# feifeibear/long-context-attention

Hardware: AMD Instinct MI355X
Metric: attention TFLOP/s (algorithmic, causal fwd+bwd) + iter ms of LongContextAttention at seqlen 64K, ulysses x ring (higher is better)
Workload: dtype bf16

## Files before the change

long-context-attention_amd/csrc/usp_flash_bwd_dq64.hip:

```cpp
#include <stdlib.h>

#include <type_traits>

#include "usp_bwd_params.hpp"
#include "usp_common.hpp"
#include "usp_hip.h"
#include "usp_mfma64.hpp"

namespace usp {

#ifndef USP_Q64_PF
#define USP_Q64_PF 3
#endif
constexpr int kQ64_PF = USP_Q64_PF;
#ifndef USP_Q64_Y1
#define USP_Q64_Y1 24
#endif
constexpr int kQ64_Y1 = USP_Q64_Y1;

#ifdef USP_Q64_TIMING
#define USP_TM(...) __VA_ARGS__
#else
#define USP_TM(...)
#endif

template <int DT, bool CAUSAL>
__global__ __launch_bounds__(256, 1) void flash_bwd_dq64_kernel(const BwdParams ) {
  using E = Elem<DT>;
  using M = M64<DT>;
  constexpr int D = 128, kBM = 256;
  constexpr int ROWB = D * 2;
  constexpr int TILEB = kTile * ROWB;
  constexpr int VOFF = 2 * TILEB;
  constexpr int NKT = D / 16, NDJ = D / 32;
  constexpr int PF = kQ64_PF;

  extern __shared__ __attribute__((aligned(16))) char smem_raw[];
  if ((uint32_t)(uintptr_t)(USP_LDS char*)smem_raw != 0u) __builtin_trap();
  USP_LDS char* smem = (USP_LDS char*)(uintptr_t)0;

  const int tid = threadIdx.x;
  const int lane = tid & 63;
  const int wave = __builtin_amdgcn_readfirstlane(tid >> 6);
  const int l31 = lane & 31;
  const int hi = lane >> 5;
  typedef const __attribute__((address_space(4))) BwdParams* KArgs;
  KArgs p = (KArgs)__builtin_amdgcn_kernarg_segment_ptr();
  asm volatile("" : "+s"(p));

  const int dma_row = lane >> 4;
  const int dma_c8 = ((lane & 15) ^ ((lane >> 4) << 2)) * 16;
  const int k_voff = dma_row * (int)p->k_ss * 2 + dma_c8, v_voff = dma_row * (int)p->v_ss * 2 + dma_c8;
  const int rd_base = l31 * ROWB + ((hi ^ tile_swz<D>(l31)) * 16);
  int tr_addr[NDJ][2];
  {
    const int i = lane & 15, grp = (lane >> 4) & 1;
#pragma unroll
    for (int dj = 0; dj < NDJ; ++dj)
#pragma unroll
      for (int e = 0; e < 2; ++e) {
        const int rr = 8 * e + 4 * hi + (i >> 2);
        const int slot = 4 * dj + 2 * grp + ((i & 3) >> 1);
        tr_addr[dj][e] = rr * ROWB + ((slot ^ tile_swz<D>(rr)) * 16) + (i & 1) * 8;
      }
  }
  const float c = p->scale_log2;

  const ItemWalk walk(p->n_items);
  for (int pass = 0;; ++pass) {
  int w = walk.at(pass);
  if (w < 0) break;
  asm volatile("" : "+s"(p));
  USP_TM(const uint64_t tm_item = __builtin_amdgcn_s_memtime();)
  w = walk.dealt(w, p->nblk);
  if (p->ksplit <= 1) w = walk.grouped(w, p->nblk, p->walk_g);
  const int qt_r = w % p->nblk;
  int rest = w / p->nblk;
  const int qt = CAUSAL ? (p->nblk - 1 - qt_r) : qt_r;
  int cut = 0;
  if (p->ksplit > 1) { cut = rest % p->ksplit; rest /= p->ksplit; }
  const int h = rest % p->Hq, b = rest / p->Hq;
  const int hkv = h / p->G;
  const int q0 = qt * kBM;
  const int qw = q0 + wave * 64;
  const int off = p->causal_off;

  int blk_kv_end = p->Sk, wave_kv_end = p->Sk;
  if (CAUSAL) {
    const int blk_last = (q0 + kBM < p->Sq ? q0 + kBM : p->Sq) - 1;
    const int wav_last = (qw + 64 < p->Sq ? qw + 64 : p->Sq) - 1;
    blk_kv_end = blk_last + off + 1 < p->Sk ? blk_last + off + 1 : p->Sk;
    wave_kv_end = wav_last + off + 1 < p->Sk ? wav_last + off + 1 : p->Sk;
  }
  if (qw >= p->Sq) wave_kv_end = 0;
  const int nt = blk_kv_end > 0 ? (blk_kv_end + kTile - 1) / kTile : 0;
  int n_full = p->Sk / kTile;
  if (CAUSAL) {
    const int lim = qw + off + 1;
    const int nf = lim > 0 ? lim / kTile : 0;
    n_full = nf < n_full ? nf : n_full;
  }
  const int n_w = wave_kv_end > 0 ? (wave_kv_end + kTile - 1) / kTile : 0;
  if (n_full > n_w) n_full = n_w;
  int tb = 0, te = nt;
  if (p->ksplit > 1) {
    const int per = (nt + p->ksplit - 1) / p->ksplit;
    tb = cut * per < nt ? cut * per : nt;
    te = tb + per < nt ? tb + per : nt;
  }
  const int e_full = n_full < tb ? tb : (n_full > te ? te : n_full);
  const int e_own = n_w < tb ? tb : (n_w > te ? te : n_w);

  u32x4 qf[2][NKT], df[2][NKT];
  float nl[2], dl[2];
#pragma unroll
  for (int qb = 0; qb < 2; ++qb) {
    const int row = qw + 32 * qb + l31;
    const int row_c = row < p->Sq ? row : p->Sq - 1;
    [[maybe_unused]] const char* qp = p->q + 2 * (b * p->q_sb + (int64_t)row_c * p->q_ss + h * p->q_sh) + 16 * hi;
    [[maybe_unused]] const char* dp = p->dout + 2 * (b * p->do_sb + (int64_t)row_c * p->do_ss + h * p->do_sh) + 16 * hi;
#if defined(__HIP_DEVICE_COMPILE__)
    asm volatile("global_load_dwordx4 %0, %16, off\n\tglobal_load_dwordx4 %1, %16, off offset:32\n\t"
                 "global_load_dwordx4 %2, %16, off offset:64\n\tglobal_load_dwordx4 %3, %16, off offset:96\n\t"
                 "global_load_dwordx4 %4, %16, off offset:128\n\tglobal_load_dwordx4 %5, %16, off offset:160\n\t"
                 "global_load_dwordx4 %6, %16, off offset:192\n\tglobal_load_dwordx4 %7, %16, off offset:224\n\t"
                 "global_load_dwordx4 %8, %17, off\n\tglobal_load_dwordx4 %9, %17, off offset:32\n\t"
                 "global_load_dwordx4 %10, %17, off offset:64\n\tglobal_load_dwordx4 %11, %17, off offset:96\n\t"
                 "global_load_dwordx4 %12, %17, off offset:128\n\tglobal_load_dwordx4 %13, %17, off offset:160\n\t"
                 "global_load_dwordx4 %14, %17, off offset:192\n\tglobal_load_dwordx4 %15, %17, off offset:224\n\t"
                 "s_waitcnt vmcnt(0)"
                 : "=&a"(qf[qb][0]), "=&a"(qf[qb][1]), "=&a"(qf[qb][2]), "=&a"(qf[qb][3]), "=&a"(qf[qb][4]), "=&a"(qf[qb][5]),
                   "=&a"(qf[qb][6]), "=&a"(qf[qb][7]), "=&a"(df[qb][0]), "=&a"(df[qb][1]), "=&a"(df[qb][2]), "=&a"(df[qb][3]),
                   "=&a"(df[qb][4]), "=&a"(df[qb][5]), "=&a"(df[qb][6]), "=&a"(df[qb][7])
                 : "v"(qp), "v"(dp) : "memory");
#endif
    const float lse = p->lse[b * p->lse_sb + h * p->lse_sh + row_c];
    const float dlt = p->delta[b * p->dl_sb + h * p->dl_sh + row_c];
    const bool live = row < p->Sq && lse != USP_NEG_INF;
    nl[qb] = live ? -lse * kLog2e : USP_NEG_INF;
    dl[qb] = live ? dlt : 0.f;
  }

  const int k_rowb = (int)p->k_ss * 2, v_rowb = (int)p->v_ss * 2;
  const int64_t k_tb = (int64_t)kTile * k_rowb, v_tb = (int64_t)kTile * v_rowb;
  int k_step = 4 * k_rowb - 1024, v_step = 4 * v_rowb - 1024;
  int lds_w = wave * 4096;
  const char* k_cur = p->k + 2 * (b * p->k_sb + hkv * p->k_sh) + (int64_t)wave * 16 * k_rowb + tb * k_tb;
  const char* v_cur = p->v + 2 * (b * p->v_sb + hkv * p->v_sh) + (int64_t)wave * 16 * v_rowb + tb * v_tb;
  int rows_kv = p->Sk - 16 * wave - tb * kTile;
  u32x4 k_rs, v_rs;
  int dma_buf = 0;
  auto dma_open = [&](int buf) {
    k_rs = make_rsrc_rows(k_cur, rows_kv, 16, k_rowb, 2 * D);
    v_rs = make_rsrc_rows(v_cur, rows_kv, 16, v_rowb, 2 * D);
    dma_buf = buf;
    k_cur += k_tb;
    v_cur += v_tb;
    rows_kv -= kTile;
  };
  auto dma_piece = [&](int n) {
    asm volatile("" : "+s"(lds_w), "+s"(k_step), "+s"(v_step));
    const int i = n & 3;
    if (n < 4) lds_dma16_asm(k_rs, lds_w + dma_buf * TILEB, k_voff ^ (16 * i), i * k_step, i);
    else lds_dma16_asm(v_rs, lds_w + VOFF + dma_buf * TILEB, v_voff ^ (16 * i), i * v_step, i);
  };

  f32x16 dq[2][NDJ];
#pragma unroll
  for (int qb = 0; qb < 2; ++qb)
#pragma unroll
    for (int dj = 0; dj < NDJ; ++dj) {
#pragma unroll
      for (int r = 0; r < 16; ++r) dq[qb][dj][r] = 0.f;
      pin_agpr(dq[qb][dj]);
    }

  dma_open(tb & 1);
#pragma unroll
  for (int n = 0; n < 8; ++n) dma_piece(n);
  dma_drain();
  __syncthreads();

  auto iter = [&](auto mask_c, int t, bool work) __attribute__((always_inline)) {
    constexpr bool MASK = decltype(mask_c)::value;
    const int par = t & 1;
    if (work) {
#pragma unroll
      for (int qb = 0; qb < 2; ++qb)
#pragma unroll
        for (int kt = 0; kt < NKT; ++kt) { pin_agpr4(qf[qb][kt]); pin_agpr4(df[qb][kt]); }
      int kr = rd_base + par * TILEB, vr = rd_base + VOFF + par * TILEB;
      asm volatile("" : "+v"(kr), "+v"(vr));
      USP_LDS const char* kt_base = smem + par * TILEB;
      f32x16 bs[2][2], bd[2][2];
      u32x4 pk[2][4];
      u32x4 ka[2 * NKT], va[2 * NKT], xa[4 * NDJ];
      auto rd_k = [&](int f) { ka[f] = *(USP_LDS const u32x4*)(smem + (f & 1) * 32 * ROWB + (kr ^ (32 * (f >> 1)))); };
      auto rd_v = [&](int f) { va[f] = *(USP_LDS const u32x4*)(smem + (f & 1) * 32 * ROWB + (vr ^ (32 * (f >> 1)))); };
      auto rd_x = [&](int f) {
        USP_LDS const char* xb = kt_base + (f / NDJ) * 16 * ROWB;
        const u32x2 a0 = lds_read_tr16(xb + tr_addr[f % NDJ][0]);
        const u32x2 a1 = lds_read_tr16(xb + tr_addr[f % NDJ][1]);
        xa[f] = u32x4{a0[0], a0[1], a1[0], a1[1]};
      };
      auto X = [&](int qb, int n) {
        const int ks = n >> 3, kb = ks >> 1, r = 8 * (ks & 1) + (n & 7);
        bs[qb][kb][r] = fast_exp2(__builtin_fmaf(bs[qb][kb][r], c, nl[qb]));
      };
      auto Y = [&](int qb, int n) {
        const int ks = n >> 3, kb = ks >> 1, r = 8 * (ks & 1) + (n & 7);
        bd[qb][kb][r] = (bd[qb][kb][r] - dl[qb]) * bs[qb][kb][r];
        if (r & 1) pk[qb][ks][(n & 7) >> 1] = E::pack2(bd[qb][kb][r - 1], bd[qb][kb][r]);
      };
      auto mask = [&](int qb) {
        const int row = qw + 32 * qb + l31;
        int klim = p->Sk - 1;
        if (CAUSAL) klim = row + off < klim ? row + off : klim;
        const int kb0 = t * kTile + 4 * hi;
#pragma unroll
        for (int r = 0; r < 16; ++r) {
          const int key = kb0 + (r & 3) + 8 * (r >> 2);
          if (key > klim) bs[qb][0][r] = USP_NEG_INF;
          if (key + 32 > klim) bs[qb][1][r] = USP_NEG_INF;
        }
      };
#pragma unroll
      for (int f = 0; f < PF; ++f) rd_k(f);
      __builtin_amdgcn_sched_barrier(0);
#pragma unroll
      for (int i = 0; i < 16; ++i) {
        const int kt = i >> 1, kb = i & 1;
        if (kt == 0) M::template s_first<MASK>(bs[0][kb], ka[i], qf[0][0]);
        else M::template s_next<MASK>(bs[0][kb], ka[i], qf[0][kt]);
        if (i == 0) { __builtin_amdgcn_sched_barrier(0); dma_open(par ^ 1); }
        if (i + PF < 16) rd_k(i + PF);
        if (i >= 1 && i <= 8) dma_piece(i - 1);
        __builtin_amdgcn_sched_barrier(0);
      }
      if (MASK) { mfma_settle(bs[0]); mask(0); }
#pragma unroll
      for (int i = 0; i < 16; ++i) {
        const int kt = i >> 1, kb = i & 1;
        if (kt == 0) M::template s_first<MASK>(bs[1][kb], ka[i], qf[1][0]);
        else M::template s_next<MASK>(bs[1][kb], ka[i], qf[1][kt]);
        if (i == 0) __builtin_amdgcn_sched_barrier(0);
        X(0, 2 * i); X(0, 2 * i + 1);
        if (i >= 16 - PF) rd_v(i - (16 - PF));
        __builtin_amdgcn_sched_barrier(0);
      }
      if (MASK) { mfma_settle(bs[1]); mask(1); }
#pragma unroll
      for (int i = 0; i < 16; ++i) {
        const int kt = i >> 1, kb = i & 1;
        if (kt == 0) M::template s_first<MASK>(bd[0][kb], va[i], df[0][0]);
        else M::template s_next<MASK>(bd[0][kb], va[i], df[0][kt]);
        if (i == 0) __builtin_amdgcn_sched_barrier(0);
        if (i + PF < 16) rd_v(i + PF);
        X(1, 2 * i); X(1, 2 * i + 1);
        __builtin_amdgcn_sched_barrier(0);
      }
#pragma unroll
      for (int i = 0; i < 16; ++i) {
        const int kt = i >> 1, kb = i & 1;
        if (kt == 0) M::template s_first<MASK>(bd[1][kb], va[i], df[1][0]);
        else M::template s_next<MASK>(bd[1][kb], va[i], df[1][kt]);
        if (i == 0) __builtin_amdgcn_sched_barrier(0);
        Y(0, 2 * i); Y(0, 2 * i + 1);
        if (i >= 16 - PF) rd_x(i - (16 - PF));
        __builtin_amdgcn_sched_barrier(0);
      }
      constexpr int NY1 = kQ64_Y1;
      static_assert(NY1 >= 16 && NY1 <= 28, "dS of k-step ks must be packed before gap 16 + 4 ks");
#pragma unroll
      for (int i = 0; i < 16; ++i) {
        M::template o_acc<MASK>(dq[0][i % NDJ], xa[i], pk[0][i / NDJ]);
        if (i == 0) __builtin_amdgcn_sched_barrier(0);
        if (i + PF < 16) rd_x(i + PF);
#pragma unroll
        for (int n = i * 32 / NY1; n < (i + 1) * 32 / NY1; ++n) Y(1, n);
        __builtin_amdgcn_sched_barrier(0);
      }
#pragma unroll
      for (int i = 0; i < 16; ++i) {
        M::template o_acc<MASK>(dq[1][i % NDJ], xa[i], pk[1][i / NDJ]);
        if (16 + i < NY1) {
#pragma unroll
          for (int n = (16 + i) * 32 / NY1; n < (16 + i + 1) * 32 / NY1; ++n) Y(1, n);
        }
        __builtin_amdgcn_sched_barrier(0);
      }
    } else {
      dma_open(par ^ 1);
#pragma unroll
      for (int n = 0; n < 8; ++n) dma_piece(n);
    }
    dma_drain();
    __syncthreads();
  };
  const std::integral_constant<bool, false> plain;
  const std::integral_constant<bool, true> masked;
  int t = tb;
  USP_TM(const uint64_t tm_loop = __builtin_amdgcn_s_memtime();)
  __builtin_amdgcn_s_waitcnt(0x0f70);
  for (; t < e_full; ++t) iter(plain, t, true);
  __builtin_amdgcn_s_waitcnt(0x0f70);
  for (; t < e_own; ++t) iter(masked, t, true);
  mfma_settle(dq);
  USP_TM(const uint64_t tm_own = __builtin_amdgcn_s_memtime(); const uint64_t tm_plain_n = n_full;)
  for (; t < te; ++t) iter(plain, t, false);
  USP_TM(const uint64_t tm_epi = __builtin_amdgcn_s_memtime();)

  mfma_settle(dq);
  asm volatile("" : "+s"(p));
  const bool wide = (p->wide16 & 1) != 0;
#pragma unroll
  for (int qb = 0; qb < 2; ++qb) {
    const int row = qw + 32 * qb + l31;
    if (wide) {
      const int row_c = row < p->Sq ? row : 0;
      store_row16_wide<E, NDJ>(p->dq16 + 2 * (b * p->dq16_sb + (int64_t)row_c * p->dq16_ss + h * p->dq16_sh), dq[qb], p->scale, hi,
                               row < p->Sq);
    } else if (row < p->Sq) {
      float* o1 = p->dq + b * p->dq_sb + (int64_t)row * p->dq_ss + h * p->dq_sh;
      char* h1 = p->dq16 ? p->dq16 + 2 * (b * p->dq16_sb + (int64_t)row * p->dq16_ss + h * p->dq16_sh) : nullptr;
      int acc_f = p->accum_dq;
      if (p->ksplit > 1) {
        o1 = p->ws_dq + ((((int64_t)cut * p->B + b) * p->Sq + row) * p->Hq + h) * D;
        h1 = nullptr;
        acc_f = 0;
      }
      const float sc = p->scale;
#pragma unroll
      for (int dj = 0; dj < NDJ; ++dj)
#pragma unroll
        for (int g4 = 0; g4 < 4; ++g4) {
          const int d0 = 32 * dj + 8 * g4 + 4 * hi;
          f32x4 v1 = {dq[qb][dj][4 * g4] * sc, dq[qb][dj][4 * g4 + 1] * sc, dq[qb][dj][4 * g4 + 2] * sc,
                      dq[qb][dj][4 * g4 + 3] * sc};
          if (acc_f) v1 += *(const f32x4*)(o1 + d0);
          if (h1) *(u32x2*)(h1 + 2 * d0) = u32x2{E::pack2(v1[0], v1[1]), E::pack2(v1[2], v1[3])};
          else *(f32x4*)(o1 + d0) = v1;
        }
    }
  }
  __syncthreads();
USP_TM(
  if (pass < 3 && lane == 0 && (blockIdx.x % 61) == 0)
    printf("TQ wg %3d pass %d wave %d qt %2d tiles own %3d (plain %3d) wg %3d : prologue %6llu own tiles %8llu (%5llu / tile) idle %6llu epilogue %6llu\n",
           (int)blockIdx.x, pass, wave, qt, n_w, (int)tm_plain_n, nt, (unsigned long long)(tm_loop - tm_item),
           (unsigned long long)(tm_own - tm_loop), (unsigned long long)((tm_own - tm_loop) / (n_w > 0 ? n_w : 1)),
           (unsigned long long)(tm_epi - tm_own), (unsigned long long)(__builtin_amdgcn_s_memtime() - tm_epi));
)
  }
}

bool dq64_serves(const BwdParams& p_in) {
  if (p_in.seq_q || p_in.seq_k || p_in.sched || p_in.win_on) return false;
  if ((p_in.k_ss * 2) % 256 != 0 || (p_in.v_ss * 2) % 256 != 0 || p_in.k_ss * 128 >= (1LL << 31) || p_in.v_ss * 128 >= (1LL << 31))
    return false;
  return true;
}

bool launch_dq64(const BwdParams& p_in, int dtype, bool causal, hipStream_t st, int* rc) {
  static const int cus = [] {
    int dev = 0, n = 0;
    if (hipGetDevice(&dev) != hipSuccess ||
        hipDeviceGetAttribute(&n, hipDeviceAttributeMultiprocessorCount, dev) != hipSuccess || n <= 0)
      n = 256;
    return n;
  }();
  if (!dq64_serves(p_in)) return false;
  BwdParams p = p_in;
  p.nblk = (p.Sq + 255) / 256;
  p.n_items = p.B * p.Hq * p.nblk * p.ksplit;
  p.wide16 = (p.ksplit <= 1 && p.dq16 && !p.accum_dq && rows16_aligned(p.dq16, p.dq16_sb, p.dq16_ss, p.dq16_sh)) ? 1 : 0;
  const int grid = (!p.interleave && p.n_items > cus) ? cus : p.n_items;
  const size_t lds = 4 * kTile * 128 * 2;
  if (dtype == USP_BF16) {
    if (causal) hipLaunchKernelGGL((flash_bwd_dq64_kernel<0, true>), dim3(grid), dim3(256), lds, st, p);
    else hipLaunchKernelGGL((flash_bwd_dq64_kernel<0, false>), dim3(grid), dim3(256), lds, st, p);
  } else {
    if (causal) hipLaunchKernelGGL((flash_bwd_dq64_kernel<1, true>), dim3(grid), dim3(256), lds, st, p);
    else hipLaunchKernelGGL((flash_bwd_dq64_kernel<1, false>), dim3(grid), dim3(256), lds, st, p);
  }
  *rc = hipGetLastError() == hipSuccess ? USP_OK : USP_ELAUNCH;
  return true;
}

}
```

Measured before the change: 1043.

## Fold delta subtraction into dP MFMA init and reschedule softmax elementwise work

The dP accumulator is now seeded with -delta through a new s_first_c MFMA variant, so the per-element dS update becomes a single multiply instead of a subtract and multiply. The exp (X) and dS (Y) elementwise work is redistributed by a generic span scheduler across the five MFMA phases, with tunable spans and a shorter default Y1 span. The aim is to cut VALU work and balance it under MFMA issue, at the cost of holding extra VGPRs for ndl and depending on s_first_c existing in the MFMA header.

```diff
diff --git a/long-context-attention_amd/csrc/usp_flash_bwd_dq64.hip b/long-context-attention_amd/csrc/usp_flash_bwd_dq64.hip
--- a/long-context-attention_amd/csrc/usp_flash_bwd_dq64.hip
+++ b/long-context-attention_amd/csrc/usp_flash_bwd_dq64.hip
@@ -13,10 +13,20 @@
 #define USP_Q64_PF 3
 #endif
 constexpr int kQ64_PF = USP_Q64_PF;
+#ifndef USP_Q64_X0
+#define USP_Q64_X0 16
+#endif
+#ifndef USP_Q64_X1
+#define USP_Q64_X1 32
+#endif
 #ifndef USP_Q64_Y1
-#define USP_Q64_Y1 24
-#endif
-constexpr int kQ64_Y1 = USP_Q64_Y1;
+#define USP_Q64_Y1 20
+#endif
+constexpr int kQ64_AT[4] = {0, 16, 32, 48};
+constexpr int kQ64_SPAN[4] = {USP_Q64_X0, USP_Q64_X1, 16, USP_Q64_Y1};
+static_assert(kQ64_SPAN[0] >= 16 && kQ64_AT[0] + kQ64_SPAN[0] <= kQ64_AT[2], "P[0] must be complete before dS[0] starts");
+static_assert(kQ64_SPAN[1] >= 16 && kQ64_AT[1] + kQ64_SPAN[1] <= kQ64_AT[3], "P[1] must be complete before dS[1] starts");
+static_assert(kQ64_SPAN[3] >= 16 && kQ64_SPAN[3] <= 28, "dS[1] of k-step ks must be packed before gap 16 + 4 ks of B6");
 
 #ifdef USP_Q64_TIMING
 #define USP_TM(...) __VA_ARGS__
@@ -113,6 +123,7 @@
 
   u32x4 qf[2][NKT], df[2][NKT];
   float nl[2], dl[2];
+  f32x16 ndl[2];
 #pragma unroll
   for (int qb = 0; qb < 2; ++qb) {
     const int row = qw + 32 * qb + l31;
@@ -139,6 +150,9 @@
     const bool live = row < p->Sq && lse != USP_NEG_INF;
     nl[qb] = live ? -lse * kLog2e : USP_NEG_INF;
     dl[qb] = live ? dlt : 0.f;
+#pragma unroll
+    for (int r = 0; r < 16; ++r) ndl[qb][r] = -dl[qb];
+    asm volatile("" : "+v"(ndl[qb]));
   }
 
   const int k_rowb = (int)p->k_ss * 2, v_rowb = (int)p->v_ss * 2;
@@ -166,12 +180,14 @@
   };
 
   f32x16 dq[2][NDJ];
+  float zero = 0.f;
+  asm volatile("" : "+v"(zero));
 #pragma unroll
   for (int qb = 0; qb < 2; ++qb)
 #pragma unroll
     for (int dj = 0; dj < NDJ; ++dj) {
 #pragma unroll
-      for (int r = 0; r < 16; ++r) dq[qb][dj][r] = 0.f;
+      for (int r = 0; r < 16; ++r) dq[qb][dj][r] = zero;
       pin_agpr(dq[qb][dj]);
     }
 
@@ -209,8 +225,20 @@
       };
       auto Y = [&](int qb, int n) {
         const int ks = n >> 3, kb = ks >> 1, r = 8 * (ks & 1) + (n & 7);
-        bd[qb][kb][r] = (bd[qb][kb][r] - dl[qb]) * bs[qb][kb][r];
+        bd[qb][kb][r] *= bs[qb][kb][r];
         if (r & 1) pk[qb][ks][(n & 7) >> 1] = E::pack2(bd[qb][kb][r - 1], bd[qb][kb][r]);
+      };
+      auto elems = [&](int g) {
+#pragma unroll
+        for (int s = 0; s < 4; ++s) {
+          const int j = g - kQ64_AT[s], sp = kQ64_SPAN[s];
+          if (j < 0 || j >= sp) continue;
+#pragma unroll
+          for (int n = j * 32 / sp; n < (j + 1) * 32 / sp; ++n) {
+            if (s < 2) X(s, n);
+            else Y(s - 2, n);
+          }
+        }
       };
       auto mask = [&](int qb) {
         const int row = qw + 32 * qb + l31;
@@ -244,7 +272,7 @@
         if (kt == 0) M::template s_first<MASK>(bs[1][kb], ka[i], qf[1][0]);
         else M::template s_next<MASK>(bs[1][kb], ka[i], qf[1][kt]);
         if (i == 0) __builtin_amdgcn_sched_barrier(0);
-        X(0, 2 * i); X(0, 2 * i + 1);
+        elems(i);
         if (i >= 16 - PF) rd_v(i - (16 - PF));
         __builtin_amdgcn_sched_barrier(0);
       }
@@ -252,41 +280,35 @@
 #pragma unroll
       for (int i = 0; i < 16; ++i) {
         const int kt = i >> 1, kb = i & 1;
-        if (kt == 0) M::template s_first<MASK>(bd[0][kb], va[i], df[0][0]);
+        if (kt == 0) M::template s_first_c<MASK>(bd[0][kb], va[i], df[0][0], ndl[0]);
         else M::template s_next<MASK>(bd[0][kb], va[i], df[0][kt]);
         if (i == 0) __builtin_amdgcn_sched_barrier(0);
         if (i + PF < 16) rd_v(i + PF);
-        X(1, 2 * i); X(1, 2 * i + 1);
+        elems(16 + i);
         __builtin_amdgcn_sched_barrier(0);
       }
 #pragma unroll
       for (int i = 0; i < 16; ++i) {
         const int kt = i >> 1, kb = i & 1;
-        if (kt == 0) M::template s_first<MASK>(bd[1][kb], va[i], df[1][0]);
+        if (kt == 0) M::template s_first_c<MASK>(bd[1][kb], va[i], df[1][0], ndl[1]);
         else M::template s_next<MASK>(bd[1][kb], va[i], df[1][kt]);
         if (i == 0) __builtin_amdgcn_sched_barrier(0);
-        Y(0, 2 * i); Y(0, 2 * i + 1);
+        elems(32 + i);
         if (i >= 16 - PF) rd_x(i - (16 - PF));
         __builtin_amdgcn_sched_barrier(0);
       }
-      constexpr int NY1 = kQ64_Y1;
-      static_assert(NY1 >= 16 && NY1 <= 28, "dS of k-step ks must be packed before gap 16 + 4 ks");
 #pragma unroll
       for (int i = 0; i < 16; ++i) {
         M::template o_acc<MASK>(dq[0][i % NDJ], xa[i], pk[0][i / NDJ]);
         if (i == 0) __builtin_amdgcn_sched_barrier(0);
         if (i + PF < 16) rd_x(i + PF);
-#pragma unroll
-        for (int n = i * 32 / NY1; n < (i + 1) * 32 / NY1; ++n) Y(1, n);
+        elems(48 + i);
         __builtin_amdgcn_sched_barrier(0);
       }
 #pragma unroll
       for (int i = 0; i < 16; ++i) {
         M::template o_acc<MASK>(dq[1][i % NDJ], xa[i], pk[1][i / NDJ]);
-        if (16 + i < NY1) {
-#pragma unroll
-          for (int n = (16 + i) * 32 / NY1; n < (16 + i + 1) * 32 / NY1; ++n) Y(1, n);
-        }
+        elems(64 + i);
         __builtin_amdgcn_sched_barrier(0);
       }
     } else {
@@ -313,12 +335,14 @@
   mfma_settle(dq);
   asm volatile("" : "+s"(p));
   const bool wide = (p->wide16 & 1) != 0;
+  int hi_e = hi;
+  asm volatile("" : "+v"(hi_e));
 #pragma unroll
   for (int qb = 0; qb < 2; ++qb) {
     const int row = qw + 32 * qb + l31;
     if (wide) {
       const int row_c = row < p->Sq ? row : 0;
-      store_row16_wide<E, NDJ>(p->dq16 + 2 * (b * p->dq16_sb + (int64_t)row_c * p->dq16_ss + h * p->dq16_sh), dq[qb], p->scale, hi,
+      store_row16_wide<E, NDJ>(p->dq16 + 2 * (b * p->dq16_sb + (int64_t)row_c * p->dq16_ss + h * p->dq16_sh), dq[qb], p->scale, hi_e,
                                row < p->Sq);
     } else if (row < p->Sq) {
       float* o1 = p->dq + b * p->dq_sb + (int64_t)row * p->dq_ss + h * p->dq_sh;
@@ -334,7 +358,7 @@
       for (int dj = 0; dj < NDJ; ++dj)
 #pragma unroll
         for (int g4 = 0; g4 < 4; ++g4) {
-          const int d0 = 32 * dj + 8 * g4 + 4 * hi;
+          const int d0 = 32 * dj + 8 * g4 + 4 * hi_e;
           f32x4 v1 = {dq[qb][dj][4 * g4] * sc, dq[qb][dj][4 * g4 + 1] * sc, dq[qb][dj][4 * g4 + 2] * sc,
                       dq[qb][dj][4 * g4 + 3] * sc};
           if (acc_f) v1 += *(const f32x4*)(o1 + d0);
```

After: 1051 (median of 6 runs). About the same (+0.8%).
